# Accenture/AmpliGraph

Hardware: AMD Instinct MI355X
Metric: training triples/sec (incl. negatives), ComplEx k=200 eta=20 FB15K-237-shaped (higher is better)
Workload: dtype f32; 1 GPU; synth-fb15k237 (uniform, seed 0) ComplEx k=200 eta=20 self_adversarial adam lr=1e-3, 10000 positives/GPU/step, tables resident in HBM, dense (non-lazy) Keras-legacy Adam every step; preset=C2, optimizer_mode=dense, deterministic=False, global_batch=10000, n_ents=14505, n_rels=237, row_floats=400, stored_row_floats=400, parallelism=single GPU

## Files before the change

### ampligraph_amd/csrc/kge_train_direct.hip

```cpp
#include "kge_train_tiled.h"

namespace kge {

constexpr int DIRECT_UN = 2;
#ifndef KGE_DIRECT_PRE
#define KGE_DIRECT_PRE 0
#endif
constexpr int DIRECT_PRE = KGE_DIRECT_PRE;
constexpr int DIRECT_PRE_N = DIRECT_PRE > 0 ? DIRECT_PRE : 1;
constexpr int DIRECT_OVF_SLACK = 256;

__host__ __device__ inline size_t direct_lds_bytes(int cap, int tile_rows) {
    const size_t n = (size_t)cap + DIRECT_OVF_SLACK;
    return n * 16 + n * 2 + (size_t)(tile_rows + 2) * 4 * 2 + (size_t)tile_rows * 2 + 64;
}

template <int MODEL, int GW>
#ifdef KGE_DIRECT_WAVES
__attribute__((amdgpu_waves_per_eu(KGE_DIRECT_WAVES, KGE_DIRECT_WAVES)))
#endif
__global__ __launch_bounds__(GW * 64) void tile_direct_kernel(TileArgs a) {
    using T = ModelTraits<MODEL>;
    constexpr int NC = T::NC;
    constexpr bool TRILINEAR = (MODEL == AMDKGE_DISTMULT || MODEL == AMDKGE_COMPLEX);
    constexpr int THREADS = GW * 64;
    extern __shared__ __attribute__((aligned(16))) char smem[];
    __shared__ int s_last, s_total, s_nact;

    const int tid = threadIdx.x, lane = tid & 63, wg = tid >> 6;
    const int tile = blockIdx.x;
    if (tile >= a.n_tiles) {
        const int64_t first = (int64_t)(tile - a.n_tiles) * THREADS + tid, stride = (int64_t)a.rel_blocks * THREADS;
        float racc;
#define KGE_REL_SWEEP(KIND) racc = opt_sweep<KIND>(a.rel_opt, first, stride)
        KGE_OPT_DISPATCH(a.rel_opt.kind, KGE_REL_SWEEP)
#undef KGE_REL_SWEEP
        if (a.rel_opt.reg_loss && a.rel_opt.lam != 0.f) {
            const float w = wave_sum(racc);
            if (lane == 0) atomicAdd(a.rel_opt.reg_loss, (double)a.rel_opt.lam * (double)w);
        }
        return;
    }
    const int cnt = min(a.counters[tile * 32], a.cap);
    const int on = min(a.counters[a.n_tiles * 32], a.ovf_cap);
    if (tid == 0)
        for (int sl = tile; sl < LOSS_PARTS; sl += a.n_tiles) {
            const unsigned long long old = atomicExch(reinterpret_cast<unsigned long long*>(a.loss_parts + (size_t)sl * LOSS_PART_STRIDE), 0ull);
            const double v = __longlong_as_double((long long)old);
            if (v != 0.0) atomicAdd(a.loss_sum, v);
        }
    const uint32_t NT = (uint32_t)a.n_tiles, RB = (uint32_t)a.rb;
    const int nrow = a.tile_rows;
    auto row_of = [&](int r) KGE_TILE_INLINE -> int64_t { return row_of_tile((uint32_t)tile, (uint32_t)r, NT, RB); };

    const int lcap = a.cap + DIRECT_OVF_SLACK;
    uint4* ents = reinterpret_cast<uint4*>(smem);
    uint16_t* order = reinterpret_cast<uint16_t*>(smem + (size_t)lcap * 16);
    int* rstart = reinterpret_cast<int*>(smem + (((size_t)lcap * 18 + 15) & ~(size_t)15));
    int* rfill = rstart + nrow + 2;
    uint16_t* active = reinterpret_cast<uint16_t*>(rfill + nrow + 2);
    const StageEntry* list = a.lists + (size_t)tile * a.cap;
    if (tid == 0) { s_total = cnt; s_nact = 0; }
    for (int r = tid; r <= nrow; r += THREADS) { rstart[r] = 0; rfill[r] = 0; }
    for (int i = tid; i < cnt; i += THREADS) ents[i] = reinterpret_cast<const uint4*>(list)[i];
    __syncthreads();
    for (int base = 0; base < on; base += THREADS) {
        uint4 e = make_uint4(0, 0, 0, 0xFFFFFFFFu);
        if (base + tid < on) e = reinterpret_cast<const uint4*>(a.ovf)[base + tid];
        if (e.w != 0xFFFFFFFFu && (e.w / RB) % NT == (uint32_t)tile) {
            const int at = atomicAdd(&s_total, 1);
            if (at < lcap) ents[at] = e;
        }
    }
    __syncthreads();
    int total = s_total;
    const bool ovf_slow = total > lcap;
    if (ovf_slow) total = cnt;
    for (int i = tid; i < total; i += THREADS) atomicAdd(&rstart[entry_local(ents[i].y) + 1], 1);
    __syncthreads();
    if (wg == 0) {
        int carry = 0;
        for (int b = 0; b <= nrow; b += 64) {
            const int r = b + lane;
            int v = (r <= nrow) ? rstart[r] : 0, s = v;
#pragma unroll
            for (int o = 1; o < 64; o <<= 1) { const int t = __shfl_up(s, o, 64); if (lane >= o) s += t; }
            if (r <= nrow) rstart[r] = carry + s;
            carry += __shfl(s, 63, 64);
        }
    }
    __syncthreads();
    for (int i = tid; i < total; i += THREADS) {
        const int lr = (int)entry_local(ents[i].y);
        order[rstart[lr] + atomicAdd(&rfill[lr], 1)] = (uint16_t)i;
    }
    if (wg == 0) {
        int n = 0;
        for (int b = 0; b < nrow; b += 64) {
            const int r = b + lane;
            bool take = false;
            if (r < nrow) {
                const int64_t row = row_of(r);
                take = row < a.n_rows;
                if (take && a.lazy && a.apply_update && !ovf_slow)
                    take = rstart[r + 1] > rstart[r] || (a.hot_map && a.hot_map[row]) || (a.touched && a.touched[row]);
            }
            const unsigned long long mk = __ballot(take);
            if (take) active[n + __builtin_amdgcn_mbcnt_hi((unsigned)(mk >> 32), __builtin_amdgcn_mbcnt_lo((unsigned)mk, 0))] = (uint16_t)r;
            n += __popcll(mk);
        }
        if (lane == 0) s_nact = n;
    }
    __syncthreads();
    const int nact = s_nact;

    const int q = lane + 64 * wg;
    const bool qok = q < a.nq;
    const int qoff = (qok ? q : 0) * 4;
    float reg_acc = 0.f;
    struct RowRegs {
        float4 x[NC], m[NC], v[NC];
        float4 sv[DIRECT_PRE_N][NC], pv[DIRECT_PRE_N];
        uint32_t meta[DIRECT_PRE_N];
        float gg[DIRECT_PRE_N];
        int e0, e1, hot, marked;
        int64_t off;
    };
    auto entry_loads = [&](int idx, uint32_t& meta, float& gg, float4 (&sv)[NC], float4& pv) KGE_TILE_INLINE {
        const uint4 e = ents[order[idx]];
        const uint32_t pos = __builtin_amdgcn_readfirstlane(e.x);
        meta = __builtin_amdgcn_readfirstlane(e.y);
        gg = __uint_as_float(__builtin_amdgcn_readfirstlane(e.z));
        const int role = meta & 3;
        const int which = (role == 0) ? 2 : (role == 1) ? 3 : (role == 2) ? 0 : 1;
        const float* src = a.stage_rows + ((int64_t)pos * a.ns + which) * a.K + qoff;
#pragma unroll
        for (int h = 0; h < NC; ++h) sv[h] = KGE_LD4(src + h * a.k);
        if constexpr (MODEL == AMDKGE_TRANSE) {
            if (role < 2) pv = KGE_LD4(a.rel + (int64_t)a.triples[3 * (int64_t)pos + 1] * a.K + qoff);
        }
    };
    auto request = [&](int i, RowRegs& R) KGE_TILE_INLINE {
        const int r = active[i];
        const int64_t row = row_of(r);
        R.e0 = rstart[r]; R.e1 = rstart[r + 1];
        R.hot = a.hot_map ? a.hot_map[row] : 0;
        R.marked = (a.touched && a.touched[row]) ? 1 : 0;
        R.off = row * a.K + qoff;
#pragma unroll
        for (int h = 0; h < NC; ++h) {
            R.m[h] = make_float4(0.f, 0.f, 0.f, 0.f); R.v[h] = R.m[h];
            R.x[h] = KGE_LD4(a.x + R.off + h * a.k);
            if (a.apply_update) {
                if (a.s0) R.m[h] = KGE_LD4(a.s0 + R.off + h * a.k);
                if (a.s1) R.v[h] = KGE_LD4(a.s1 + R.off + h * a.k);
            }
        }
#pragma unroll
        for (int u = 0; u < DIRECT_PRE; ++u)
            if (R.e0 + u < R.e1) entry_loads(R.e0 + u, R.meta[u], R.gg[u], R.sv[u], R.pv[u]);
    };
    auto fold = [&](uint32_t meta, float ge, const float4 (&sv)[NC], const float4& pv, const float4 (&x)[NC], float4 (&g)[NC]) KGE_TILE_INLINE {
        const int role = meta & 3;
        if (TRILINEAR || role >= 2) {
#pragma unroll
            for (int h = 0; h < NC; ++h) {
                g[h].x += ge * sv[h].x; g[h].y += ge * sv[h].y; g[h].z += ge * sv[h].z; g[h].w += ge * sv[h].w;
            }
        } else if constexpr (MODEL == AMDKGE_ROTATE) {
#pragma unroll
            for (int c = 0; c < 4; ++c) {
                const float dr = (&x[0].x)[c] - (&sv[0].x)[c], di = (&x[NC - 1].x)[c] - (&sv[NC - 1].x)[c];
                const float mm = KGE_SQRT(dr * dr + di * di) + ((qoff + c >= a.k_live) ? 1.f : 0.f);
                const float gm = KGE_DIV(ge, mm);
                (&g[0].x)[c] += gm * dr;
                (&g[NC - 1].x)[c] += gm * di;
            }
        } else if constexpr (MODEL == AMDKGE_TRANSE) {
#pragma unroll
            for (int c = 0; c < 4; ++c) {
                float p[1] = {(&pv.x)[c]}, e[1] = {(&x[0].x)[c]}, sd[1] = {(&sv[0].x)[c]}, ds[1], dp[1], dd[1];
                if (role == 0) grad_unit<AMDKGE_TRANSE>(sd, p, e, ge, ds, dp, dd);
                else grad_unit<AMDKGE_TRANSE>(e, p, sd, ge, ds, dp, dd);
                (&g[0].x)[c] += (role == 0) ? dd[0] : ds[0];
            }
        }
    };
    RowRegs cur, nxt;
    if (nact > 0) request(0, cur);
    for (int i = 0; i < nact; ++i) {
        if (i + 1 < nact) request(i + 1, nxt);
        float4 g[NC];
#pragma unroll
        for (int h = 0; h < NC; ++h) g[h] = make_float4(0.f, 0.f, 0.f, 0.f);
#pragma unroll
        for (int u = 0; u < DIRECT_PRE; ++u)
            if (cur.e0 + u < cur.e1) fold(cur.meta[u], cur.gg[u], cur.sv[u], cur.pv[u], cur.x, g);
        for (int i0 = cur.e0 + DIRECT_PRE; i0 < cur.e1; i0 += DIRECT_UN) {
            uint32_t meta[DIRECT_UN];
            float gg[DIRECT_UN];
            float4 sv[DIRECT_UN][NC], pv[DIRECT_UN];
#pragma unroll
            for (int u = 0; u < DIRECT_UN; ++u)
                if (i0 + u < cur.e1) entry_loads(i0 + u, meta[u], gg[u], sv[u], pv[u]);
#pragma unroll
            for (int u = 0; u < DIRECT_UN; ++u)
                if (i0 + u < cur.e1) fold(meta[u], gg[u], sv[u], pv[u], cur.x, g);
        }
        bool row_touched = cur.e1 > cur.e0 || cur.hot || cur.marked;
        if (ovf_slow) {
            const uint32_t row32 = (uint32_t)((cur.off - qoff) / a.K);
            for (int base = 0; base < on; base += 64) {
                uint4 e = make_uint4(0, 0, 0, 0xFFFFFFFFu);
                if (base + lane < on) e = reinterpret_cast<const uint4*>(a.ovf)[base + lane];
                unsigned long long mk = __ballot(e.w == row32);
                row_touched = row_touched || mk != 0ull;
                while (mk) {
                    const int tt = __builtin_ctzll(mk);
                    mk &= mk - 1;
                    const uint32_t pos = __builtin_amdgcn_readlane(e.x, tt), meta = __builtin_amdgcn_readlane(e.y, tt);
                    const float ge = __uint_as_float(__builtin_amdgcn_readlane(e.z, tt));
                    const int role = meta & 3, which = (role == 0) ? 2 : (role == 1) ? 3 : (role == 2) ? 0 : 1;
                    const float* src = a.stage_rows + ((int64_t)pos * a.ns + which) * a.K + qoff;
                    float4 sv[NC], pv = make_float4(0.f, 0.f, 0.f, 0.f);
#pragma unroll
                    for (int h = 0; h < NC; ++h) sv[h] = KGE_LD4(src + h * a.k);
                    if constexpr (MODEL == AMDKGE_TRANSE) {
                        if (role < 2) pv = KGE_LD4(a.rel + (int64_t)a.triples[3 * (int64_t)pos + 1] * a.K + qoff);
                    }
                    fold(meta, ge, sv, pv, cur.x, g);
                }
            }
        }
        if (qok && !(a.lazy && a.apply_update && !row_touched)) {
            const int64_t off = cur.off;
            const int hot = cur.hot;
#pragma unroll
            for (int h = 0; h < NC; ++h) {
                float4* gp4 = (a.pos_atomic || !a.apply_update) ? reinterpret_cast<float4*>(a.g_ent + off + h * a.k) : nullptr;
                if (hot) {
                    float4* hp = reinterpret_cast<float4*>(a.hot_buf + (int64_t)(hot - 1) * HOT_REPL * a.K + qoff + h * a.k);
#pragma unroll 4
                    for (int rp = 0; rp < HOT_REPL; ++rp) {
                        const float4 t = hp[(size_t)rp * (a.K >> 2)];
                        g[h].x += t.x; g[h].y += t.y; g[h].z += t.z; g[h].w += t.w;
                        hp[(size_t)rp * (a.K >> 2)] = make_float4(0.f, 0.f, 0.f, 0.f);
                    }
                }
                if (a.pos_atomic) {
                    const float4 gd = *gp4;
                    g[h].x += gd.x; g[h].y += gd.y; g[h].z += gd.z; g[h].w += gd.w;
                    if (a.apply_update) *gp4 = make_float4(0.f, 0.f, 0.f, 0.f);
                }
                if (!a.apply_update) {
                    *gp4 = g[h];
                    continue;
                }
#define KGE_UPD(KIND) do { \
                    opt_elem<KIND>(a.opt, cur.x[h].x, g[h].x, cur.m[h].x, cur.v[h].x, reg_acc); opt_elem<KIND>(a.opt, cur.x[h].y, g[h].y, cur.m[h].y, cur.v[h].y, reg_acc); \
                    opt_elem<KIND>(a.opt, cur.x[h].z, g[h].z, cur.m[h].z, cur.v[h].z, reg_acc); opt_elem<KIND>(a.opt, cur.x[h].w, g[h].w, cur.m[h].w, cur.v[h].w, reg_acc); \
                    if constexpr (opt_nslots(KIND) >= 1) *reinterpret_cast<float4*>(a.s0 + off + h * a.k) = cur.m[h]; \
                    if constexpr (opt_nslots(KIND) == 2) *reinterpret_cast<float4*>(a.s1 + off + h * a.k) = cur.v[h]; } while (0)
                KGE_OPT_DISPATCH(a.opt.kind, KGE_UPD)
#undef KGE_UPD
                *reinterpret_cast<float4*>(a.x + off + h * a.k) = cur.x[h];
            }
        }
        cur = nxt;
    }
    if (a.apply_update && a.reg_loss && a.opt.lam != 0.f) {
        const float w = wave_sum(reg_acc);
        if (lane == 0) atomicAdd(a.loss_parts + (size_t)((tile * GW + wg) & (LOSS_PARTS - 1)) * LOSS_PART_STRIDE + 1, (double)a.opt.lam * (double)w);
    }
    __syncthreads();
    if (a.touched)
        for (int r = tid; r < nrow; r += THREADS)
            if (row_of(r) < a.n_rows) a.touched[row_of(r)] = 0;
    if (tid == 0) {
        a.counters[tile * 32] = 0;
        __threadfence();
        s_last = 0;
        if (atomicAdd(a.counters + (size_t)(a.n_tiles + 1) * 32, 1) == a.n_tiles - 1) {
            a.counters[a.n_tiles * 32] = 0;
            a.counters[(a.n_tiles + 1) * 32] = 0;
            s_last = 1;
        }
    }
    __syncthreads();
    if (s_last && wg == 0 && a.apply_update && a.reg_loss && a.opt.lam != 0.f) fold_loss_parts(a.loss_parts, a.reg_loss, lane, 1);
}

template <int MODEL>
static int launch_direct(const TileArgs& te, hipStream_t st) {
    const size_t sh = direct_lds_bytes(te.cap, te.tile_rows);
    if (te.nq <= 128) return set_error(AMDKGE_EUNSUPPORTED, "tile_direct: rows of up to 128 quads per half take the LDS-accumulator tiles");
    if (te.gw == 4) hipLaunchKernelGGL((tile_direct_kernel<MODEL, 4>), dim3(te.n_tiles + te.rel_blocks), dim3(256), sh, st, te);
    else hipLaunchKernelGGL((tile_direct_kernel<MODEL, 8>), dim3(te.n_tiles + te.rel_blocks), dim3(512), sh, st, te);
    return check_launch("tile_direct");
}

int run_tile_direct(int model, const TileArgs& te, hipStream_t st) {
#define KGE_RUN(MODEL) return launch_direct<MODEL>(te, st)
    KGE_MODEL_DISPATCH(model, KGE_RUN)
#undef KGE_RUN
}

}
```

### ampligraph_amd/csrc/kge_train_tile.hip

```cpp
#include <type_traits>
#include "kge_train_tiled.h"

namespace kge {

template <int MODEL, int CH, int UNROLL, bool DET = false>
__global__ __launch_bounds__(TILE_THREADS) void tile_backward_kernel(TileArgs a) {
    using T = ModelTraits<MODEL>;
    constexpr int NC = T::NC;
    constexpr bool TRILINEAR = (MODEL == AMDKGE_DISTMULT || MODEL == AMDKGE_COMPLEX);
    extern __shared__ __attribute__((aligned(16))) char smem[];
    float* acc = reinterpret_cast<float*>(smem);

    __shared__ int s_last;
    const int tid = threadIdx.x, lane = tid & 63, wv = tid >> 6;
    const int tile = blockIdx.x;
    if (tile >= a.n_tiles) {
        const int64_t first = (int64_t)(tile - a.n_tiles) * TILE_THREADS + tid, stride = (int64_t)a.rel_blocks * TILE_THREADS;
        float racc;
#define KGE_REL_SWEEP(KIND) racc = opt_sweep<KIND>(a.rel_opt, first, stride)
        KGE_OPT_DISPATCH(a.rel_opt.kind, KGE_REL_SWEEP)
#undef KGE_REL_SWEEP
        if (a.rel_opt.reg_loss && a.rel_opt.lam != 0.f) {
            const float w = wave_sum(racc);
            if (lane == 0) atomicAdd(a.rel_opt.reg_loss, (double)a.rel_opt.lam * (double)w);
        }
        return;
    }
    const int cnt = KGE_DBG(a, 4096) ? 0 : min(a.counters[tile * 32], a.cap);
    const int on = KGE_DBG(a, 4096) ? 0 : min(a.counters[a.n_tiles * 32], a.ovf_cap);
    if (tid == 0)
        for (int sl = tile; sl < LOSS_PARTS; sl += a.n_tiles) {
            const unsigned long long old = atomicExch(reinterpret_cast<unsigned long long*>(a.loss_parts + (size_t)sl * LOSS_PART_STRIDE), 0ull);
            const double v = __longlong_as_double((long long)old);
            if (v != 0.0) atomicAdd(a.loss_sum, v);
        }
    const uint32_t NT = (uint32_t)a.n_tiles;
    const int nrow = a.tile_rows;
    const uint32_t RB = (uint32_t)a.rb;
    auto row_of = [&](int r) KGE_TILE_INLINE -> int64_t { return row_of_tile((uint32_t)tile, (uint32_t)r, NT, RB); };
    auto row_ok = [&](int r) KGE_TILE_INLINE -> bool { return row_of(r) < a.n_rows; };

    const int gw = a.gw, grp = wv / gw, wg = wv % gw, G = TILE_WAVES / gw;
    bool qok[CH];
    int qoff[CH];
#pragma unroll
    for (int c = 0; c < CH; ++c) {
        const int q = lane + 64 * c + 64 * CH * wg;
        qok[c] = q < a.nq;
        qoff[c] = (qok[c] ? q : 0) * 4;
    }
    float* own = acc + (size_t)a.tile_rows * a.K;
    const size_t acc_floats = (size_t)a.tile_rows * a.K * (a.own_cache ? 2 : 1);
    for (int r = grp; r < (KGE_DBG(a, 2048) ? 0 : nrow); r += G)
#pragma unroll
        for (int c = 0; c < CH; ++c)
#pragma unroll
            for (int h = 0; h < NC; ++h)
                if (qok[c]) {
                    *reinterpret_cast<float4*>(acc + (size_t)r * a.K + qoff[c] + h * a.k) = make_float4(0, 0, 0, 0);
                    if constexpr (MODEL == AMDKGE_ROTATE) {
                        if (a.own_cache && row_ok(r))
                            *reinterpret_cast<float4*>(own + (size_t)r * a.K + qoff[c] + h * a.k) = KGE_LD4(a.x + row_of(r) * a.K + qoff[c] + h * a.k);
                    }
                }
    uint8_t* tflag = reinterpret_cast<uint8_t*>(acc + acc_floats);
    if (a.lazy)
        for (int r = grp + G * lane; r < nrow; r += G * 64)
            tflag[r * gw + wg] = (a.touched && row_ok(r) && a.touched[row_of(r)]) ? 1 : 0;

    constexpr int NX = TRILINEAR ? 1 : NC;
    auto load_ops = [&](uint32_t pos, uint32_t meta, int pp, float4 (&v)[CH][NC], float4 (&pv)[CH][NX], float4 (&ev)[CH][NX], auto own_c) KGE_TILE_INLINE {
        constexpr bool OWN = decltype(own_c)::value;
        const int role = meta & 3;
        const int which = (role == 0) ? 2 : (role == 1) ? 3 : (role == 2) ? 0 : 1;
        const float* src = a.stage_rows + ((int64_t)pos * a.ns + which) * a.K;
#pragma unroll
        for (int c = 0; c < CH; ++c)
#pragma unroll
            for (int h = 0; h < NC; ++h) v[c][h] = *reinterpret_cast<const float4*>(src + qoff[c] + h * a.k);
        if constexpr (!TRILINEAR) {
            if (role < 2) {
                if constexpr (OWN) {
                } else {
                    const float* re = a.x + row_of((int)entry_local(meta)) * a.K;
#pragma unroll
                    for (int c = 0; c < CH; ++c)
#pragma unroll
                        for (int h = 0; h < NC; ++h) ev[c][h] = KGE_LD4(re + qoff[c] + h * a.k);
                }
                if constexpr (MODEL != AMDKGE_ROTATE) {
                    const float* rp = a.rel + (int64_t)pp * a.K;
#pragma unroll
                    for (int c = 0; c < CH; ++c)
#pragma unroll
                        for (int h = 0; h < NC; ++h) pv[c][h] = KGE_LD4(rp + qoff[c] + h * a.k);
                }
            }
        }
    };
    auto add_entry = [&](uint32_t meta, float g, const float4 (&v)[CH][NC], const float4 (&pv)[CH][NX], const float4 (&ev)[CH][NX], auto own_c) KGE_TILE_INLINE {
        constexpr bool OWN = decltype(own_c)::value;
        const int role = meta & 3;
        const int lr = (int)entry_local(meta);
        float* arow = acc + (size_t)lr * a.K;
        if (a.lazy) tflag[lr * gw + wg] = 1;
        float4 out[CH][NC];
        if (TRILINEAR || role >= 2) {
#pragma unroll
            for (int c = 0; c < CH; ++c)
#pragma unroll
                for (int h = 0; h < NC; ++h) out[c][h] = make_float4(g * v[c][h].x, g * v[c][h].y, g * v[c][h].z, g * v[c][h].w);
        } else if constexpr (MODEL == AMDKGE_ROTATE) {
            float4 eo[CH][NC];
#pragma unroll
            for (int c = 0; c < CH; ++c)
#pragma unroll
                for (int h = 0; h < NC; ++h)
                    if constexpr (OWN) eo[c][h] = *reinterpret_cast<const float4*>(own + (size_t)lr * a.K + qoff[c] + h * a.k);
                    else eo[c][h] = ev[c][h < NX ? h : 0];
#pragma unroll
            for (int c = 0; c < CH; ++c)
#pragma unroll
                for (int u = 0; u < 4; ++u) {
                    const float dr = (&eo[c][0].x)[u] - (&v[c][0].x)[u], di = (&eo[c][1].x)[u] - (&v[c][1].x)[u];
                    const float m = kge_sqrt_t<DET>(dr * dr + di * di) + ((qoff[c] + u >= a.k_live) ? 1.f : 0.f);
                    const float gm = kge_div_t<DET>(g, m);
                    (&out[c][0].x)[u] = gm * dr;
                    (&out[c][1].x)[u] = gm * di;
                }
        } else {
#pragma unroll
            for (int c = 0; c < CH; ++c) {
#pragma unroll
                for (int u = 0; u < 4; ++u) {
                    float p[NC], e[NC], sd[NC], ds[NC], dp[NC], dd[NC];
#pragma unroll
                    for (int h = 0; h < NC; ++h) {
                        p[h] = (&pv[c][h < NX ? h : 0].x)[u]; e[h] = (&ev[c][h < NX ? h : 0].x)[u]; sd[h] = (&v[c][h].x)[u];
                    }
                    if constexpr (MODEL != AMDKGE_ROTATE) prep_rel<MODEL>(a.mc, p);
                    const float pad1 = (MODEL == AMDKGE_ROTATE && qoff[c] + u >= a.k_live) ? 1.f : 0.f;
                    if (role == 0) grad_unit<MODEL>(sd, p, e, g, ds, dp, dd, pad1);
                    else grad_unit<MODEL>(e, p, sd, g, ds, dp, dd, pad1);
#pragma unroll
                    for (int h = 0; h < NC; ++h) (&out[c][h].x)[u] = (role == 0) ? dd[h] : ds[h];
                }
            }
        }
#pragma unroll
        for (int c = 0; c < CH; ++c) {
            if (!qok[c]) continue;
#pragma unroll
            for (int h = 0; h < NC; ++h) {
                float4* d = reinterpret_cast<float4*>(arow + qoff[c] + h * a.k);
                float4 t = *d;
                t.x += out[c][h].x; t.y += out[c][h].y; t.z += out[c][h].z; t.w += out[c][h].w;
                *d = t;
            }
        }
    };
    auto process = [&](const StageEntry& mine, unsigned long long mask) KGE_TILE_INLINE {
        int mine_pp = 0;
        if constexpr (MODEL == AMDKGE_TRANSE) {
            if (mask) mine_pp = a.triples[3 * (int64_t)mine.pos + 1];
        }
        while (mask) {
            uint32_t meta[UNROLL];
            float g[UNROLL];
            float4 v[UNROLL][CH][NC], pv[UNROLL][CH][NX], ev[UNROLL][CH][NX];
            int m = 0;
#pragma unroll
            for (int u = 0; u < UNROLL; ++u) {
                if (mask) {
                    const int tt = __builtin_ctzll(mask);
                    mask &= mask - 1;
                    const uint32_t pos = __builtin_amdgcn_readlane(mine.pos, tt);
                    meta[u] = __builtin_amdgcn_readlane(mine.meta, tt);
                    g[u] = __int_as_float(__builtin_amdgcn_readlane(__float_as_int(mine.g), tt));
                    load_ops(pos, meta[u], __builtin_amdgcn_readlane(mine_pp, tt), v[u], pv[u], ev[u], std::false_type{});
                    m = u + 1;
                }
            }
#pragma unroll
            for (int u = 0; u < UNROLL; ++u)
                if (u < m) add_entry(meta[u], g[u], v[u], pv[u], ev[u], std::false_type{});
        }
    };

    const StageEntry* list = a.lists + (size_t)tile * a.cap;
    if (a.det) {
        uint4* sbuf = reinterpret_cast<uint4*>(smem + (((size_t)a.tile_rows * a.K * 4 + (size_t)a.tile_rows * gw + 15) & ~(size_t)15));
        __shared__ int s_total;
        if (tid == 0) s_total = cnt;
        for (int i = tid; i < cnt && i < a.sort_cap; i += TILE_THREADS) sbuf[i] = reinterpret_cast<const uint4*>(list)[i];
        __syncthreads();
        for (int base = 0; base < on; base += TILE_THREADS) {
            uint4 e = make_uint4(0, 0, 0, 0xFFFFFFFFu);
            if (base + tid < on) e = reinterpret_cast<const uint4*>(a.ovf)[base + tid];
            if (e.w != 0xFFFFFFFFu && (e.w / RB) % NT == (uint32_t)tile) {
                const int at = atomicAdd(&s_total, 1);
                if (at < a.sort_cap) sbuf[at] = e;
            }
        }
        __syncthreads();
        int total = s_total;
        if (total > a.sort_cap) {
            if (tid == 0) atomicExch(a.status_flag, 1);
            total = a.sort_cap;
        }
        {
            __shared__ int s_qovf;
            if (tid == 0) s_qovf = 0;
            __syncthreads();
            const int qstride = a.sort_cap / 8;
            int QC = 64;
            while (QC * 2 <= min(256, qstride)) QC *= 2;
            uint16_t* qix = reinterpret_cast<uint16_t*>(sbuf + a.sort_cap) + (size_t)wv * qstride;
            int qn = 0;
            bool over = qstride < 64;
            for (int base = 0; base < total && !over; base += 64) {
                const bool in = base + lane < total;
                const uint32_t meta = in ? sbuf[base + lane].y : 0u;
                const bool mineq = in && (int)(entry_local(meta) % G) == grp;
                const unsigned long long m = __ballot(mineq);
                const int c = __popcll(m);
                if (qn + c > QC) { over = true; break; }
                if (mineq) qix[qn + __builtin_amdgcn_mbcnt_hi((unsigned)(m >> 32), __builtin_amdgcn_mbcnt_lo((unsigned)m, 0))] = (uint16_t)(base + lane);
                qn += c;
            }
            if (over && lane == 0) s_qovf = 1;
            __syncthreads();
            if (!s_qovf && !KGE_DBG(a, 16384)) {
                int n2w = 64;
                while (n2w < qn) n2w <<= 1;
                for (int i = qn + lane; i < n2w; i += 64) qix[i] = 0xFFFFu;
                __builtin_amdgcn_fence(__ATOMIC_ACQ_REL, "wavefront"); __builtin_amdgcn_wave_barrier();
                auto key_less = [&](uint16_t ix, uint16_t iy) KGE_TILE_INLINE -> bool {
                    if (iy == 0xFFFFu) return ix != 0xFFFFu;
                    if (ix == 0xFFFFu) return false;
                    const uint4 x = sbuf[ix], y = sbuf[iy];
                    if (x.x != y.x) return x.x < y.x;
                    if (x.y != y.y) return x.y < y.y;
                    if (x.z != y.z) return x.z < y.z;
                    if (x.w != y.w) return x.w < y.w;
                    return ix < iy;
                };
                for (int kk = 2; kk <= n2w; kk <<= 1)
                    for (int j = kk >> 1; j > 0; j >>= 1) {
                        for (int i = lane; i < n2w; i += 64) {
                            const int pi = i ^ j;
                            if (pi > i) {
                                const uint16_t x = qix[i], y = qix[pi];
                                const bool up = (i & kk) == 0;
                                if (up ? key_less(y, x) : key_less(x, y)) { qix[i] = y; qix[pi] = x; }
                            }
                        }
                        __builtin_amdgcn_fence(__ATOMIC_ACQ_REL, "wavefront"); __builtin_amdgcn_wave_barrier();
                    }
                for (int base = 0; base < qn; base += 64) {
                    StageEntry mine{0u, 0u, 0.f, 0u};
                    const bool in = base + lane < qn;
                    if (in) { const uint4 e = sbuf[qix[base + lane]]; mine = StageEntry{e.x, e.y, __uint_as_float(e.z), e.w}; }
                    process(mine, __ballot(in));
                }
            } else {
        uint16_t* idxA = reinterpret_cast<uint16_t*>(sbuf + a.sort_cap);
        uint16_t* idxB = idxA + a.sort_cap;
        int* ccnt = reinterpret_cast<int*>(idxB + a.sort_cap);
        __shared__ int s_ones;
        const int nchunk = (total + 63) >> 6;
        for (int i = tid; i < total; i += TILE_THREADS) idxA[i] = (uint16_t)i;
        __syncthreads();
        constexpr int SORT_IT = 8;
        for (int bit = 0; bit < (KGE_DBG(a, 16384) ? 0 : a.pos_bits); ++bit) {
            int myid[SORT_IT], mybit[SORT_IT], myin[SORT_IT];
#pragma unroll
            for (int it = 0; it < SORT_IT; ++it) {
                const int e = tid + it * TILE_THREADS;
                myid[it] = 0; mybit[it] = 0; myin[it] = 0;
                if ((e & ~63) < total) {
                    const bool valid = e < total;
                    myid[it] = valid ? idxA[e] : 0;
                    mybit[it] = valid ? (int)((sbuf[myid[it]].x >> bit) & 1u) : 0;
                    const unsigned long long m = __ballot(mybit[it] != 0);
                    myin[it] = __builtin_amdgcn_mbcnt_hi((unsigned)(m >> 32), __builtin_amdgcn_mbcnt_lo((unsigned)m, 0));
                    if (lane == 0) ccnt[e >> 6] = __popcll(m);
                }
            }
            __syncthreads();
            if (wv == 0) {
                int carry = 0;
                for (int c0 = 0; c0 < nchunk; c0 += 64) {
                    const int c = c0 + lane;
                    const int v = c < nchunk ? ccnt[c] : 0;
                    int incl = v;
#pragma unroll
                    for (int o = 1; o < 64; o <<= 1) { const int t = __shfl_up(incl, o, 64); if (lane >= o) incl += t; }
                    if (c < nchunk) ccnt[c] = carry + incl - v;
                    carry += __shfl(incl, 63, 64);
                }
                if (lane == 0) s_ones = carry;
            }
            __syncthreads();
            const int zeros = total - s_ones;
#pragma unroll
            for (int it = 0; it < SORT_IT; ++it) {
                const int e = tid + it * TILE_THREADS;
                if (e < total) {
                    const int ones_before = ccnt[e >> 6] + myin[it];
                    idxB[mybit[it] ? zeros + ones_before : e - ones_before] = (uint16_t)myid[it];
                }
            }
            __syncthreads();
            uint16_t* t = idxA; idxA = idxB; idxB = t;
        }
        if (!KGE_DBG(a, 16384)) {
            for (int i = tid; i < total; i += TILE_THREADS) {
                const uint4 me = sbuf[idxA[i]];
                int gs = i;
                while (gs > 0 && sbuf[idxA[gs - 1]].x == me.x) --gs;
                int r = 0;
                for (int j = gs; j < total; ++j) {
                    if (j == i) continue;
                    const uint4 y = sbuf[idxA[j]];
                    if (y.x != me.x) break;
                    const bool lt = (y.y != me.y) ? (y.y < me.y) : ((y.z != me.z) ? (y.z < me.z) : ((y.w != me.w) ? (y.w < me.w) : (j < i)));
                    r += lt ? 1 : 0;
                }
                idxB[gs + r] = idxA[i];
            }
            __syncthreads();
            uint16_t* t = idxA; idxA = idxB; idxB = t;
        }
        for (int base = 0; base < total; base += 64) {
            StageEntry mine{0u, 0u, 0.f, 0u};
            const bool in = base + lane < total;
            if (in) { const uint4 e = sbuf[idxA[base + lane]]; mine = StageEntry{e.x, e.y, __uint_as_float(e.z), e.w}; }
            process(mine, __ballot(in && (int)(entry_local(mine.meta) % G) == grp));
        }
            }
        }
    } else if (!tile_queued(MODEL, CH, a.K)) {
        for (int base = 0; base < cnt; base += 64) {
            StageEntry mine{0u, 0u, 0.f, 0u};
            const bool in = base + lane < cnt;
            if (in) mine = list[base + lane];
            process(mine, __ballot(in && (int)(entry_local(mine.meta) % G) == grp));
        }
        for (int base = 0; base < on; base += 64) {
            StageEntry mine{0u, 0u, 0.f, 0xFFFFFFFFu};
            if (base + lane < on) mine = a.ovf[base + lane];
            const bool hit = mine.dest != 0xFFFFFFFFu && (mine.dest / RB) % NT == (uint32_t)tile;
            process(mine, __ballot(hit && (int)(entry_local(mine.meta) % G) == grp));
        }
    } else {
    uint4* queue = reinterpret_cast<uint4*>(smem + ((acc_floats * 4 + (a.lazy ? (size_t)a.tile_rows * gw : 0) + 15) & ~(size_t)15)) +
                   (size_t)wv * TILE_QCAP;
    int qn = 0;
    auto drain_n = [&](auto n_c, auto own_c, const uint4* q) KGE_TILE_INLINE {
        constexpr int UN = decltype(n_c)::value;
        for (int i0 = 0; i0 < qn; i0 += UN) {
            uint32_t meta[UN];
            float g[UN];
            float4 v[UN][CH][NC], pv[UN][CH][NX], ev[UN][CH][NX];
#pragma unroll
            for (int u = 0; u < UN; ++u) {
                if (i0 + u < qn) {
                    const uint4 e = q[i0 + u];
                    meta[u] = __builtin_amdgcn_readfirstlane(e.y);
                    g[u] = __uint_as_float(__builtin_amdgcn_readfirstlane(e.z));
                    load_ops(__builtin_amdgcn_readfirstlane(e.x), meta[u], (int)__builtin_amdgcn_readfirstlane(e.w), v[u], pv[u], ev[u], own_c);
                }
            }
#pragma unroll
            for (int u = 0; u < UN; ++u)
                if (i0 + u < qn) add_entry(meta[u], g[u], v[u], pv[u], ev[u], own_c);
        }
        qn = 0;
    };
    auto drain = [&](const uint4* q) KGE_TILE_INLINE {
        if constexpr (MODEL == AMDKGE_ROTATE) {
            if (a.own_cache) { drain_n(std::integral_constant<int, UNROLL>{}, std::true_type{}, q); return; }
        }
        drain_n(std::integral_constant<int, UNROLL>{}, std::false_type{}, q);
    };
    if constexpr (MODEL != AMDKGE_TRANSE) {
        auto collect = [&](const StageEntry& mine, bool sel) KGE_TILE_INLINE {
            const unsigned long long mask = __ballot(sel);
            if (!mask) return;
            if (qn + 64 > TILE_QCAP) drain(queue);
            if (sel) {
                uint32_t pp = 0;
                if constexpr (MODEL == AMDKGE_TRANSE) pp = (uint32_t)a.triples[3 * (int64_t)mine.pos + 1];
                queue[qn + __builtin_amdgcn_mbcnt_hi((unsigned)(mask >> 32), __builtin_amdgcn_mbcnt_lo((unsigned)mask, 0))] =
                    make_uint4(mine.pos, mine.meta, __float_as_uint(mine.g), pp);
            }
            qn += __popcll(mask);
        };
        {
            StageEntry next{0u, 0u, 0.f, 0u};
            if (lane < cnt) next = list[lane];
            for (int base = 0; base < cnt; base += 64) {
                const StageEntry mine = next;
                const bool in = base + lane < cnt;
                if (base + 64 + lane < cnt) next = list[base + 64 + lane];
                collect(mine, in && (int)(entry_local(mine.meta) % G) == grp);
            }
        }
        for (int base = 0; base < on; base += 64) {
            StageEntry mine{0u, 0u, 0.f, 0xFFFFFFFFu};
            if (base + lane < on) mine = a.ovf[base + lane];
            const bool hit = mine.dest != 0xFFFFFFFFu && (mine.dest / RB) % NT == (uint32_t)tile;
            collect(mine, hit && (int)(entry_local(mine.meta) % G) == grp);
        }
        drain(queue);
    } else {
    constexpr int TILE_QFAST = 64, FAST_U = 16;
    const bool coded = a.sign_codes != nullptr;
    uint4* const queue_slow = coded ? queue + TILE_QFAST : queue;
    const int slow_cap = coded ? TILE_QCAP - TILE_QFAST : TILE_QCAP;
    int qf = 0;
    uint32_t padfill[CH];
#pragma unroll
    for (int c = 0; c < CH; ++c) {
        padfill[c] = 0u;
#pragma unroll
        for (int x = 0; x < 4; ++x) padfill[c] |= (qoff[c] + x >= a.k_live) ? (1u << (8 * x)) : 0u;
    }
    auto drain_fast = [&]() KGE_TILE_INLINE {
        {
            for (int i0 = 0; i0 < qf; i0 += FAST_U) {
                uint32_t meta[FAST_U], gb[FAST_U], cw[FAST_U][CH];
                uint32_t redo = 0u;
#pragma unroll
                for (int u = 0; u < FAST_U; ++u) {
                    if (i0 + u < qf) {
                        const uint4 e = queue[i0 + u];
                        meta[u] = __builtin_amdgcn_readfirstlane(e.y);
                        gb[u] = __builtin_amdgcn_readfirstlane(e.z);
                        const uint32_t* src = a.sign_codes + ((int64_t)__builtin_amdgcn_readfirstlane(e.x) * a.eta + (meta[u] >> ENTRY_J_SHIFT)) * a.nq;
#pragma unroll
                        for (int c = 0; c < CH; ++c) cw[u][c] = src[qoff[c] >> 2];
                    }
                }
#pragma unroll
                for (int u = 0; u < FAST_U; ++u) {
                    if (i0 + u < qf) {
                        bool tiny = false;
#pragma unroll
                        for (int c = 0; c < CH; ++c) {
                            const uint32_t t = (cw[u][c] & 0x7f7f7f7fu) | padfill[c];
                            const uint32_t t7 = t ^ 0x7f7f7f7fu;
                            tiny |= qok[c] && ((((t - 0x01010101u) & ~t) | ((t7 - 0x01010101u) & ~t7)) & 0x80808080u) != 0u;
                        }
                        if (__ballot(tiny)) {
                            redo |= 1u << u;
                            continue;
                        }
                        const int lr = (int)entry_local(meta[u]);
                        float* arow = acc + (size_t)lr * a.K;
                        if (a.lazy) tflag[lr * gw + wg] = 1;
                        const unsigned g2 = (meta[u] & 3u) == 0u ? gb[u] ^ 0x80000000u : gb[u];
#pragma unroll
                        for (int c = 0; c < CH; ++c) {
                            if (!qok[c]) continue;
                            float4* dst = reinterpret_cast<float4*>(arow + qoff[c]);
                            float4 t = *dst;
#pragma unroll
                            for (int x = 0; x < 4; ++x) {
                                const float y = __uint_as_float(__builtin_amdgcn_bitop3_b32(cw[u][c] << (24 - 8 * x), 0x80000000u, g2, 0x6a));
                                (&t.x)[x] += (qoff[c] + x < a.k_live) ? y : 0.f;
                            }
                            *dst = t;
                        }
                    }
                }
                while (redo) {
                    const int u = __builtin_ctz(redo);
                    redo &= redo - 1;
                    const uint4 e = queue[i0 + u];
                    const uint32_t pos = __builtin_amdgcn_readfirstlane(e.x), m16 = __builtin_amdgcn_readfirstlane(e.y) & 0xFFFFu;
                    float4 v1[CH][NC], pv1[CH][NX], ev1[CH][NX];
                    load_ops(pos, m16, a.triples[3 * (int64_t)pos + 1], v1, pv1, ev1, std::false_type{});
                    add_entry(m16, __uint_as_float(__builtin_amdgcn_readfirstlane(e.z)), v1, pv1, ev1, std::false_type{});
                }
            }
        }
        qf = 0;
    };
    const int nb = (cnt + 63) >> 6, nch = nb + ((on + 63) >> 6);
    auto load_chunk = [&](int it) KGE_TILE_INLINE -> StageEntry {
        StageEntry en{0u, 0u, 0.f, 0xFFFFFFFFu};
        if (it < nb) { if (it * 64 + lane < cnt) en = list[it * 64 + lane]; }
        else if (it < nch) { if ((it - nb) * 64 + lane < on) en = a.ovf[(it - nb) * 64 + lane]; }
        return en;
    };
    StageEntry next = load_chunk(0);
    for (int it = 0; it <= nch; ++it) {
        const StageEntry mine = next;
        next = load_chunk(it + 1);
        bool sel = mine.dest != 0xFFFFFFFFu && (int)(entry_local(mine.meta) % G) == grp;
        if (it >= nb) sel = sel && (mine.dest / RB) % NT == (uint32_t)tile;
        const bool fast = coded && sel && (mine.meta & 3u) < 2u;
        sel = sel && !fast;
        const unsigned long long mf = __ballot(fast), ms = __ballot(sel);
        const int nf = __popcll(mf), ns = __popcll(ms);
#ifdef KGE_DRAIN_EARLY
        if (it == nch || qf + 64 > TILE_QFAST || qn + 64 > slow_cap) {
#else
        if (it == nch || qf + nf > TILE_QFAST || qn + ns > slow_cap) {
#endif
            drain_fast();
            drain(queue_slow);
        }
        if (fast) queue[qf + __builtin_amdgcn_mbcnt_hi((unsigned)(mf >> 32), __builtin_amdgcn_mbcnt_lo((unsigned)mf, 0))] =
                      make_uint4(mine.pos, mine.meta, __float_as_uint(mine.g), 0u);
        qf += nf;
        if (sel) {
            uint32_t pp = 0;
            if constexpr (!TRILINEAR) {
                if (!coded) pp = (uint32_t)a.triples[3 * (int64_t)mine.pos + 1];
            }
            queue_slow[qn + __builtin_amdgcn_mbcnt_hi((unsigned)(ms >> 32), __builtin_amdgcn_mbcnt_lo((unsigned)ms, 0))] =
                make_uint4(mine.pos, mine.meta, __float_as_uint(mine.g), pp);
        }
        qn += ns;
    }
    }
    }

    float reg_acc = 0.f;
    auto flush = [&](auto kind_c) KGE_TILE_INLINE {
    constexpr int KIND = decltype(kind_c)::value;
    for (int r = grp; r < (KGE_DBG(a, 1024) ? 0 : nrow); r += G) {
        const float* arow = acc + (size_t)r * a.K;
        if (!row_ok(r)) continue;
        const int hot = a.hot_map ? a.hot_map[row_of(r)] : 0;
        if (a.lazy && a.apply_update && !hot && !tflag[r * gw + wg]) continue;
        float4 gq[CH][NC], xq[CH][NC], mq[CH][NC], vq[CH][NC];
#pragma unroll
        for (int c = 0; c < CH; ++c) {
            if (!qok[c]) continue;
#pragma unroll
            for (int h = 0; h < NC; ++h) {
                float4 g = *reinterpret_cast<const float4*>(arow + qoff[c] + h * a.k);
                const int64_t off = row_of(r) * a.K + qoff[c] + h * a.k;
                float4* gp4 = reinterpret_cast<float4*>(a.g_ent + off);
                if (hot) {
                    float4* hp = reinterpret_cast<float4*>(a.hot_buf + (int64_t)(hot - 1) * HOT_REPL * a.K + qoff[c] + h * a.k);
#pragma unroll 4
                    for (int q = 0; q < HOT_REPL; ++q) {
                        const float4 t = hp[(size_t)q * (a.K >> 2)];
                        g.x += t.x; g.y += t.y; g.z += t.z; g.w += t.w;
                        hp[(size_t)q * (a.K >> 2)] = make_float4(0.f, 0.f, 0.f, 0.f);
                    }
                }
                if (a.pos_atomic) {
                    const float4 gd = *gp4;
                    g.x += gd.x; g.y += gd.y; g.z += gd.z; g.w += gd.w;
                    if (a.apply_update) *gp4 = make_float4(0.f, 0.f, 0.f, 0.f);
                }
                gq[c][h] = g;
                xq[c][h] = make_float4(0, 0, 0, 0); mq[c][h] = xq[c][h]; vq[c][h] = xq[c][h];
                if (!a.apply_update) {
                    *gp4 = g;
                    continue;
                }
                xq[c][h] = *reinterpret_cast<const float4*>(a.x + off);
                if constexpr (opt_nslots(KIND) >= 1) mq[c][h] = *reinterpret_cast<const float4*>(a.s0 + off);
                if constexpr (opt_nslots(KIND) == 2) vq[c][h] = *reinterpret_cast<const float4*>(a.s1 + off);
            }
        }
        if (!a.apply_update) continue;
#pragma unroll
        for (int c = 0; c < CH; ++c) {
            if (!qok[c]) continue;
#pragma unroll
            for (int h = 0; h < NC; ++h) {
                const int64_t off = row_of(r) * a.K + qoff[c] + h * a.k;
                float4 x = xq[c][h], m = mq[c][h], v = vq[c][h];
                const float4 g = gq[c][h];
                opt_elem<KIND>(a.opt, x.x, g.x, m.x, v.x, reg_acc); opt_elem<KIND>(a.opt, x.y, g.y, m.y, v.y, reg_acc);
                opt_elem<KIND>(a.opt, x.z, g.z, m.z, v.z, reg_acc); opt_elem<KIND>(a.opt, x.w, g.w, m.w, v.w, reg_acc);
                if constexpr (opt_nslots(KIND) >= 1) *reinterpret_cast<float4*>(a.s0 + off) = m;
                if constexpr (opt_nslots(KIND) == 2) *reinterpret_cast<float4*>(a.s1 + off) = v;
                *reinterpret_cast<float4*>(a.x + off) = x;
            }
        }
    }
    };
#define KGE_FLUSH(KIND) flush(std::integral_constant<int, KIND>{})
    KGE_OPT_DISPATCH(a.opt.kind, KGE_FLUSH)
#undef KGE_FLUSH
    if (a.apply_update && a.reg_loss && a.opt.lam != 0.f) {
        const float w = wave_sum(reg_acc);
        if (lane == 0) atomicAdd(a.loss_parts + (size_t)((tile * TILE_WAVES + wv) & (LOSS_PARTS - 1)) * LOSS_PART_STRIDE + 1, (double)a.opt.lam * (double)w);
    }
    __syncthreads();
    if (a.touched)
        for (int r = tid; r < nrow; r += TILE_THREADS)
            if (row_ok(r)) a.touched[row_of(r)] = 0;
    if (tid == 0) {
        a.counters[tile * 32] = 0;
        __threadfence();
        s_last = 0;
        if (atomicAdd(a.counters + (size_t)(a.n_tiles + 1) * 32, 1) == a.n_tiles - 1) {
            a.counters[a.n_tiles * 32] = 0;
            a.counters[(a.n_tiles + 1) * 32] = 0;
            s_last = 1;
        }
    }
    __syncthreads();
    if (s_last && wv == 0 && a.apply_update && a.reg_loss && a.opt.lam != 0.f) fold_loss_parts(a.loss_parts, a.reg_loss, lane, 1);
}

template <int MODEL, int CH, int UNROLL, bool DET = false>
static int launch_tile(const TileArgs& a, size_t shmem, hipStream_t st) {
    static PerDeviceOnce attr;
    if (int rc = ensure_dynamic_lds(attr, {(const void*)tile_backward_kernel<MODEL, CH, UNROLL, DET>}, 160 * 1024 - 256,
                                    "tile_backward")) return rc;
    hipLaunchKernelGGL((tile_backward_kernel<MODEL, CH, UNROLL, DET>), dim3(a.n_tiles + a.rel_blocks), dim3(TILE_THREADS), shmem, st, a);
    return check_launch("tile_backward");
}

template <int MODEL>
static int tile_by_width(const TileArgs& te, hipStream_t st) {
    constexpr bool TRILINEAR = (MODEL == AMDKGE_DISTMULT || MODEL == AMDKGE_COMPLEX);
    const size_t shmem_t = te.det ? (((size_t)te.tile_rows * te.K * 4 + (size_t)te.tile_rows * te.gw + 15) & ~(size_t)15) + (size_t)te.sort_cap * 20 + 1024
                                  : (((size_t)te.tile_rows * te.K * 4 * (te.own_cache ? 2 : 1) + (te.lazy ? (size_t)te.tile_rows * te.gw : 0) + 15) & ~(size_t)15) +
                                        (tile_queued(MODEL, tile_ch_of(te.nq), te.K) ? TILE_QUEUE_BYTES : 0);
    constexpr int U1 = TRILINEAR ? 8 : 4;
    constexpr int U2 = TRILINEAR ? 4 : 2;
    if constexpr (MODEL == AMDKGE_ROTATE) {
        if (te.det) {
            if (te.nq <= 64 || te.nq > 128) return launch_tile<MODEL, 1, U1, true>(te, shmem_t, st);
            return launch_tile<MODEL, 2, U2, true>(te, shmem_t, st);
        }
    }
    if (te.nq <= 64 || te.nq > 128) return launch_tile<MODEL, 1, U1>(te, shmem_t, st);
    return launch_tile<MODEL, 2, U2>(te, shmem_t, st);
}

int run_tile_backward(int model, const TileArgs& te, hipStream_t st) {
#define KGE_RUN(MODEL) return tile_by_width<MODEL>(te, st)
    KGE_MODEL_DISPATCH(model, KGE_RUN)
#undef KGE_RUN
}

}
```

Baseline: 1.489 billion triples/s.

## Move loss-part fold to relation block and release tile counters early

Tiles no longer serialize a loop of atomicExch/atomicAdd on the loss slots at kernel start. The first relation-optimizer block folds them with a wave-parallel reduction instead, or tiles fold them at the end when there are no relation blocks. When no regularization fold is needed, each tile resets its counter, takes its completion ticket, and clears touched flags right after loading its list, then exits without the tail barrier and threadfence. This shortens the critical path at the start and end of each tile. It relies on the counters and touched flags not being read later in the same kernel, and adds an explicit s_waitcnt so the reset happens after the reads.

```diff
diff --git a/ampligraph_amd/csrc/kge_train_direct.hip b/ampligraph_amd/csrc/kge_train_direct.hip
--- a/ampligraph_amd/csrc/kge_train_direct.hip
+++ b/ampligraph_amd/csrc/kge_train_direct.hip
@@ -31,6 +31,7 @@
     const int tile = blockIdx.x;
     if (tile >= a.n_tiles) {
         const int64_t first = (int64_t)(tile - a.n_tiles) * THREADS + tid, stride = (int64_t)a.rel_blocks * THREADS;
+        if (tile == a.n_tiles && wg == 0) fold_loss_parts(a.loss_parts, a.loss_sum, lane);
         float racc;
 #define KGE_REL_SWEEP(KIND) racc = opt_sweep<KIND>(a.rel_opt, first, stride)
         KGE_OPT_DISPATCH(a.rel_opt.kind, KGE_REL_SWEEP)
@@ -43,12 +44,7 @@
     }
     const int cnt = min(a.counters[tile * 32], a.cap);
     const int on = min(a.counters[a.n_tiles * 32], a.ovf_cap);
-    if (tid == 0)
-        for (int sl = tile; sl < LOSS_PARTS; sl += a.n_tiles) {
-            const unsigned long long old = atomicExch(reinterpret_cast<unsigned long long*>(a.loss_parts + (size_t)sl * LOSS_PART_STRIDE), 0ull);
-            const double v = __longlong_as_double((long long)old);
-            if (v != 0.0) atomicAdd(a.loss_sum, v);
-        }
+    const bool reg_fold = a.apply_update && a.reg_loss && a.opt.lam != 0.f;
     const uint32_t NT = (uint32_t)a.n_tiles, RB = (uint32_t)a.rb;
     const int nrow = a.tile_rows;
     auto row_of = [&](int r) KGE_TILE_INLINE -> int64_t { return row_of_tile((uint32_t)tile, (uint32_t)r, NT, RB); };
@@ -63,7 +59,13 @@
     if (tid == 0) { s_total = cnt; s_nact = 0; }
     for (int r = tid; r <= nrow; r += THREADS) { rstart[r] = 0; rfill[r] = 0; }
     for (int i = tid; i < cnt; i += THREADS) ents[i] = reinterpret_cast<const uint4*>(list)[i];
-    __syncthreads();
+    asm volatile("s_waitcnt vmcnt(0) lgkmcnt(0)" ::"v"(cnt), "v"(on) : "memory");
+    __syncthreads();
+    int ticket = -1;
+    if (!reg_fold && tid == 0) {
+        a.counters[tile * 32] = 0;
+        ticket = atomicAdd(a.counters + (size_t)(a.n_tiles + 1) * 32, 1);
+    }
     for (int base = 0; base < on; base += THREADS) {
         uint4 e = make_uint4(0, 0, 0, 0xFFFFFFFFu);
         if (base + tid < on) e = reinterpret_cast<const uint4*>(a.ovf)[base + tid];
@@ -272,6 +274,24 @@
         const float w = wave_sum(reg_acc);
         if (lane == 0) atomicAdd(a.loss_parts + (size_t)((tile * GW + wg) & (LOSS_PARTS - 1)) * LOSS_PART_STRIDE + 1, (double)a.opt.lam * (double)w);
     }
+    if (a.rel_blocks == 0 && tid == 0)
+        for (int sl = tile; sl < LOSS_PARTS; sl += a.n_tiles) {
+            const unsigned long long old = atomicExch(reinterpret_cast<unsigned long long*>(a.loss_parts + (size_t)sl * LOSS_PART_STRIDE), 0ull);
+            const double v = __longlong_as_double((long long)old);
+            if (v != 0.0) atomicAdd(a.loss_sum, v);
+        }
+    if (!reg_fold) {
+        if (a.touched) {
+            __syncthreads();
+            for (int r = tid; r < nrow; r += THREADS)
+                if (row_of(r) < a.n_rows) a.touched[row_of(r)] = 0;
+        }
+        if (tid == 0 && ticket == a.n_tiles - 1) {
+            a.counters[a.n_tiles * 32] = 0;
+            a.counters[(a.n_tiles + 1) * 32] = 0;
+        }
+        return;
+    }
     __syncthreads();
     if (a.touched)
         for (int r = tid; r < nrow; r += THREADS)
@@ -287,7 +307,7 @@
         }
     }
     __syncthreads();
-    if (s_last && wg == 0 && a.apply_update && a.reg_loss && a.opt.lam != 0.f) fold_loss_parts(a.loss_parts, a.reg_loss, lane, 1);
+    if (s_last && wg == 0) fold_loss_parts(a.loss_parts, a.reg_loss, lane, 1);
 }
 
 template <int MODEL>
diff --git a/ampligraph_amd/csrc/kge_train_tile.hip b/ampligraph_amd/csrc/kge_train_tile.hip
--- a/ampligraph_amd/csrc/kge_train_tile.hip
+++ b/ampligraph_amd/csrc/kge_train_tile.hip
@@ -16,6 +16,7 @@
     const int tile = blockIdx.x;
     if (tile >= a.n_tiles) {
         const int64_t first = (int64_t)(tile - a.n_tiles) * TILE_THREADS + tid, stride = (int64_t)a.rel_blocks * TILE_THREADS;
+        if (tile == a.n_tiles && wv == 0) fold_loss_parts(a.loss_parts, a.loss_sum, lane);
         float racc;
 #define KGE_REL_SWEEP(KIND) racc = opt_sweep<KIND>(a.rel_opt, first, stride)
         KGE_OPT_DISPATCH(a.rel_opt.kind, KGE_REL_SWEEP)
@@ -28,12 +29,7 @@
     }
     const int cnt = KGE_DBG(a, 4096) ? 0 : min(a.counters[tile * 32], a.cap);
     const int on = KGE_DBG(a, 4096) ? 0 : min(a.counters[a.n_tiles * 32], a.ovf_cap);
-    if (tid == 0)
-        for (int sl = tile; sl < LOSS_PARTS; sl += a.n_tiles) {
-            const unsigned long long old = atomicExch(reinterpret_cast<unsigned long long*>(a.loss_parts + (size_t)sl * LOSS_PART_STRIDE), 0ull);
-            const double v = __longlong_as_double((long long)old);
-            if (v != 0.0) atomicAdd(a.loss_sum, v);
-        }
+    const bool reg_fold = a.apply_update && a.reg_loss && a.opt.lam != 0.f;
     const uint32_t NT = (uint32_t)a.n_tiles;
     const int nrow = a.tile_rows;
     const uint32_t RB = (uint32_t)a.rb;
@@ -67,6 +63,19 @@
     if (a.lazy)
         for (int r = grp + G * lane; r < nrow; r += G * 64)
             tflag[r * gw + wg] = (a.touched && row_ok(r) && a.touched[row_of(r)]) ? 1 : 0;
+
+    int ticket = -1;
+    if (!reg_fold) {
+        asm volatile("s_waitcnt vmcnt(0) lgkmcnt(0)" ::"v"(cnt), "v"(on) : "memory");
+        __syncthreads();
+        if (tid == 0) {
+            a.counters[tile * 32] = 0;
+            ticket = atomicAdd(a.counters + (size_t)(a.n_tiles + 1) * 32, 1);
+        }
+        if (a.touched)
+            for (int r = tid; r < nrow; r += TILE_THREADS)
+                if (row_ok(r)) a.touched[row_of(r)] = 0;
+    }
 
     constexpr int NX = TRILINEAR ? 1 : NC;
     auto load_ops = [&](uint32_t pos, uint32_t meta, int pp, float4 (&v)[CH][NC], float4 (&pv)[CH][NX], float4 (&ev)[CH][NX], auto own_c) KGE_TILE_INLINE {
@@ -596,6 +605,19 @@
         const float w = wave_sum(reg_acc);
         if (lane == 0) atomicAdd(a.loss_parts + (size_t)((tile * TILE_WAVES + wv) & (LOSS_PARTS - 1)) * LOSS_PART_STRIDE + 1, (double)a.opt.lam * (double)w);
     }
+    if (a.rel_blocks == 0 && tid == TILE_THREADS - 64)
+        for (int sl = tile; sl < LOSS_PARTS; sl += a.n_tiles) {
+            const unsigned long long old = atomicExch(reinterpret_cast<unsigned long long*>(a.loss_parts + (size_t)sl * LOSS_PART_STRIDE), 0ull);
+            const double v = __longlong_as_double((long long)old);
+            if (v != 0.0) atomicAdd(a.loss_sum, v);
+        }
+    if (!reg_fold) {
+        if (tid == 0 && ticket == a.n_tiles - 1) {
+            a.counters[a.n_tiles * 32] = 0;
+            a.counters[(a.n_tiles + 1) * 32] = 0;
+        }
+        return;
+    }
     __syncthreads();
     if (a.touched)
         for (int r = tid; r < nrow; r += TILE_THREADS)
@@ -611,7 +633,7 @@
         }
     }
     __syncthreads();
-    if (s_last && wv == 0 && a.apply_update && a.reg_loss && a.opt.lam != 0.f) fold_loss_parts(a.loss_parts, a.reg_loss, lane, 1);
+    if (s_last && wv == 0) fold_loss_parts(a.loss_parts, a.reg_loss, lane, 1);
 }
 
 template <int MODEL, int CH, int UNROLL, bool DET = false>
```

New measurement: 1.542 billion triples/s (median of 6 runs). 3.5% higher.
